# msmbuilder/msmbuilder

Hardware: AMD Instinct MI355X
Metric: frames/sec tICA fit + KCenters assign, 10M x 512 feats (higher is better)
Workload: dtype f32

## Files before the change

### msmbuilder_amd/csrc/distance_kcbatch_dev.h

```cpp
#pragma once
#include "common.h"
#include "distance_dev.h"

namespace msm {

constexpr int KCB_JMAX = 32, KCB_CAP = 2048, KCB_NLEV = 6, KCB_TARGET = 1536;
template <int CTRL>
__device__ __forceinline__ double kcb_dpp_f64(double v)
{
    const int lo = __builtin_amdgcn_update_dpp(0, __double2loint(v), CTRL, 0xf, 0xf, false);
    const int hi = __builtin_amdgcn_update_dpp(0, __double2hiint(v), CTRL, 0xf, 0xf, false);
    return __hiloint2double(hi, lo);
}
__device__ __forceinline__ double kcb_readlane_f64(double v, int lane)
{
    return __hiloint2double(__builtin_amdgcn_readlane(__double2hiint(v), lane), __builtin_amdgcn_readlane(__double2loint(v), lane));
}
__device__ __forceinline__ void kcb_wave_argmax(double v, long long i, double& ov, long long& oi)
{
    const double w = i >= 0 ? v : -1.0;
    double x = w;
    x = fmax(x, kcb_dpp_f64<0xB1>(x));
    x = fmax(x, kcb_dpp_f64<0x4E>(x));
    x = fmax(x, kcb_dpp_f64<0x141>(x));
// ... 163 lines not shown
        }
        if (th > vl) th = vl;
        S->theta = th;
        S->count = 0;
        for (int q = 0; q < KCB_NLEV; ++q) S->lev[q] = 0;
        S->J = J;
        S->k_done = k0 + J;
        S->rounds += 1;
        S->fallbacks += fell;
    }
}

constexpr int KCB_CAPR = 1024, KCB_HDR = 48, KCB_LEV0 = 32;
__host__ __device__ constexpr size_t kcb_rec_doubles(long long m) { return (size_t)KCB_HDR + (size_t)KCB_CAPR * (size_t)(2 + m); }

__global__ void kcb_boot_records_kernel(const double* __restrict__ cands, int world, long long m, double* __restrict__ recs)
{
    const int r = blockIdx.x, tid = threadIdx.x;
    if (r >= world) return;
    const double* c = cands + (size_t)r * (2 + m);
    double* o = recs + (size_t)r * kcb_rec_doubles(m);
    if (tid < KCB_HDR) {
        double v = 0.0;
        if (tid == 8) v = c[0];
        else if (tid == 9) v = c[1];
        else if (tid >= 10 && tid < 10 + 16) v = tid - 10 < m ? c[2 + tid - 10] : 0.0;
        o[tid] = v;
    }
}

template <int NP>
__global__ __launch_bounds__(DT) void kcb_pack_kernel(KscArgs P, KcbState* S, double* __restrict__ rec)
{
    __shared__ double rv[DT];
    __shared__ long long ri[DT];
    const int tid = threadIdx.x, m = (int)P.m;
    if (S->J == 0) return;
    double bv = -1.0;
    long long bi = -1;
    for (int k = tid; k < P.nblk; k += DT) {
        const KcPartial q = P.next[k];
        if (q.i >= 0 && (bi < 0 || kc_better(q.v, q.i, bv, bi))) {
            bv = q.v;
            bi = q.i;
        }
    }
    rv[tid] = bv;
    ri[tid] = bi;
    __syncthreads();
    for (int k = DT / 2; k > 0; k >>= 1) {
        if (tid < k) {
            const long long oi = ri[tid + k];
            if (oi >= 0 && (ri[tid] < 0 || kc_better(rv[tid + k], oi, rv[tid], ri[tid]))) {
                rv[tid] = rv[tid + k];
                ri[tid] = oi;
            }
        }
        __syncthreads();
    }
    const long long w = ri[0];
    const unsigned cnt = S->count;
    if (tid < KCB_HDR) {
        double v = 0.0;
        if (tid == 0) v = (double)cnt;
        else if (tid > KCB_LEV0 && tid < KCB_LEV0 + KCB_NLEV) v = (double)S->lev[tid - KCB_LEV0];
        else if (tid == 8) v = w >= 0 ? rv[0] : -1.0;
        else if (tid == 9) v = w >= 0 ? (double)(P.row_offset + w) : -1.0;
        else if (tid >= 10 && tid < 26) v = (w >= 0 && tid - 10 < m) ? P.X[w * P.m + (tid - 10)] : 0.0;
        rec[tid] = v;
    }
    const unsigned ne = cnt <= (unsigned)KCB_CAPR ? cnt : 0u;
    for (unsigned e = tid; e < ne; e += DT) {
        const long long p = S->list[e];
        double* o = rec + KCB_HDR + (size_t)e * (2 + m);
        o[0] = P.dist[p];
        o[1] = (double)(P.row_offset + p);
        for (int f = 0; f < m; ++f) o[2 + f] = P.X[p * P.m + f];
    }
}

template <int NP>
__global__ __launch_bounds__(DT) void kcenters_batch_pass_kernel(KscArgs P, KcbState* S)
{
    constexpr int R = 2;
    constexpr int NW = ksc_words(NP, 2), RW = NW + 1;
    constexpr int SB = 2 * NP;
    typedef float f32x2 __attribute__((ext_vector_type(2)));
    __shared__ __attribute__((aligned(16))) f32x2 ycf[KCB_JMAX][NP];
    __shared__ double yd[KCB_JMAX][2 * NP];
    __shared__ float epsb[KCB_JMAX];
    __shared__ double rv[DT];
    __shared__ long long ri[DT];
    __shared__ unsigned slev[KCB_NLEV];
    const int tid = threadIdx.x, m = (int)P.m;
    const int J = S->J;
    if (J == 0) return;
    const int kbase = S->k_done - J;
    const float theta = S->theta;
    const long long ntile = (P.n + (long long)R * DT - 1) / ((long long)R * DT);
    unsigned qn[R][RW];
    auto load_tile = [&](long long t) {
#pragma unroll
        for (int k = 0; k < R; ++k) {
            const long long p0 = t * (R * DT) + k * DT + tid;
            const long long pc = p0 < P.n ? p0 : P.n - 1;
            const unsigned* xr = static_cast<const unsigned*>(P.xs) + pc * RW;
            if ((RW & 3) == 0) {
#pragma unroll
                for (int j = 0; j < RW / 4; ++j) {
                    const uint4 v = reinterpret_cast<const uint4*>(xr)[j];
                    qn[k][4 * j] = v.x;
                    qn[k][4 * j + 1] = v.y;
                    qn[k][4 * j + 2] = v.z;
                    qn[k][4 * j + 3] = v.w;
                }
            } else if ((RW & 1) == 0) {
#pragma unroll
                for (int j = 0; j < RW / 2; ++j) {
                    const uint2 v = reinterpret_cast<const uint2*>(xr)[j];
                    qn[k][2 * j] = v.x;
                    qn[k][2 * j + 1] = v.y;
                }
            } else {
#pragma unroll
                for (int j = 0; j < RW; ++j) qn[k][j] = xr[j];
            }
        }
    };
    if ((long long)blockIdx.x < ntile) load_tile(blockIdx.x);
    if (tid < KCB_NLEV) slev[tid] = 0;
    for (int e = tid; e < KCB_JMAX * 2 * NP; e += DT) {
        const int j = e / (2 * NP), f = e - j * (2 * NP);
        const double y = j < J ? S->cen[j][f] : 0.0;
        yd[j][f] = y;
        reinterpret_cast<float*>(&ycf[j][0])[f] = (float)(y - (f < m ? P.c0[f] : 0.0));
    }
    if (tid < KCB_JMAX) {
        double c0n2 = 0.0, yn2 = 0.0, ycn2 = 0.0;
        for (int f = 0; f < 2 * NP; ++f) {
            const double y = tid < J ? S->cen[tid][f] : 0.0, c0f = f < m ? P.c0[f] : 0.0;
            c0n2 = fma(c0f, c0f, c0n2);
            yn2 = fma(y, y, yn2);
            ycn2 = fma(y - c0f, y - c0f, ycn2);
        }
        const double g2 = __longlong_as_double((long long)P.gmax2[0]), r2 = __longlong_as_double((long long)P.gmax2[1]);
        double eps0 = (sqrt(r2) + sqrt(yn2) + 2.0 * sqrt(c0n2)) * 0x1p-48 + 1e-37;
        if (!(g2 < 1e36) || !(r2 < 1e76) || !(ycn2 < 1e36)) eps0 = NAN;
        epsb[tid] = fmaf(0x1p-19f, (float)(sqrt(ycn2) * 1.000001), (float)(eps0 * 1.000001));
    }
    __syncthreads();
    constexpr float E32 = 0x1p-19f;
    constexpr float QSQ = NP == 1 ? 1.4143f : NP == 2 ? 2.f : NP == 3 ? 2.4495f : NP == 4 ? 2.8285f : NP == 5 ? 3.1623f
                        : NP == 6 ? 3.4642f : NP == 7 ? 3.7417f : 4.f;
    constexpr float QA = 0.51f * 1.02f * QSQ + E32 * 127.f * QSQ * 1.001f;
    float bf = -1.f;
    long long bi = -1;
    double bx = 0.0;
    bool bknown = false;
    unsigned nlev[KCB_NLEV];
#pragma unroll
    for (int l = 0; l < KCB_NLEV; ++l) nlev[l] = 0;
    for (long long t = blockIdx.x; t < ntile; t += gridDim.x) {
        float cf[R];
        unsigned cmask[R];
        long long pr[R];
        unsigned q[R][RW];
#pragma unroll
        for (int k = 0; k < R; ++k) {
            pr[k] = t * (R * DT) + k * DT + tid;
#pragma unroll
            for (int j = 0; j < RW; ++j) q[k][j] = qn[k][j];
            cf[k] = __uint_as_float(q[k][NW]);
        }
        if (t + gridDim.x < ntile) load_tile(t + gridDim.x);
#pragma unroll
        for (int k = 0; k < R; ++k) {
            const float sf = __uint_as_float(((q[k][SB >> 2] >> (8 * (SB & 3))) & 0xffffu) << 16);
            f32x2 xt[NP];
#pragma unroll
            for (int g = 0; g < NP; ++g) {
                xt[g].x = (float)((int)(q[k][(2 * g) >> 2] << (24 - 8 * ((2 * g) & 3))) >> 24) * sf;
                xt[g].y = (float)((int)(q[k][(2 * g + 1) >> 2] << (24 - 8 * ((2 * g + 1) & 3))) >> 24) * sf;
            }
            const float base = cf[k] + sf * QA;
            unsigned mk = 0;
            for (int j = 0; j < J; ++j) {
                f32x2 acc = {0.f, 0.f};
#pragma unroll
                for (int g = 0; g < NP; ++g) {
                    const f32x2 d = xt[g] - ycf[j][g];
                    acc = __builtin_elementwise_fma(d, d, acc);
                }
                const float T = (base + epsb[j]) * (1.f + 0x1p-20f);
                if (!(acc.x + acc.y >= T * T)) mk |= 1u << j;
            }
            cmask[k] = pr[k] < P.n ? mk : 0u;
        }
        if (cmask[0] | cmask[1]) {
            double x[R][2 * NP], cur[R];
#pragma unroll
            for (int k = 0; k < R; ++k) {
                const long long pc = pr[k] < P.n ? pr[k] : P.n - 1;
                const double* xp = P.X + pc * P.m;
                if (P.vecw == 16 && (m & 1) == 0) {
#pragma unroll
                    for (int j = 0; j < NP; ++j) {
                        const raw_f32x4 v = *reinterpret_cast<const raw_f32x4*>(xp + 2 * j);
                        x[k][2 * j] = reinterpret_cast<const double*>(&v)[0];
                        x[k][2 * j + 1] = reinterpret_cast<const double*>(&v)[1];
                    }
                } else {
#pragma unroll
                    for (int f = 0; f < 2 * NP; ++f) x[k][f] = xp[f < m ? f : m - 1];
#pragma unroll
                    for (int f = 0; f < 2 * NP; ++f)
                        if (f >= m) x[k][f] = 0.0;
                }
                cur[k] = P.dist[pc];
            }
#pragma unroll
            for (int k = 0; k < R; ++k) {
                unsigned mk = cmask[k];
                int lab = -1;
                double c = cur[k];
                while (mk) {
                    const int j = __builtin_ctz(mk);
                    mk &= mk - 1;
                    double a = 0.0, b = 0.0;
#pragma unroll
                    for (int f = 0; f < 2 * NP; ++f) m_update<double, M_EUCLIDEAN>(a, b, x[k][f], yd[j][f]);
                    const double d = m_final<M_EUCLIDEAN>(a, b, P.m);
                    if (d < c) {
                        c = d;
                        lab = kbase + j;
                    }
                }
                if (lab >= 0) {
                    P.dist[pr[k]] = c;
                    P.labels[pr[k]] = lab;
                    cf[k] = ksc_round_up(c);
                    static_cast<unsigned*>(P.xs)[pr[k] * RW + NW] = __float_as_uint(cf[k]);
                }
            }
        }
#pragma unroll
        for (int k = 0; k < R; ++k) {
            const long long p = pr[k];
            const bool in = p < P.n;
            const bool lst = in && cf[k] > theta;
            const unsigned long long bal = __builtin_amdgcn_ballot_w64(lst);
            if (bal) {
                const int lane = tid & 63, leader = __builtin_ctzll(bal);
                unsigned base = 0;
                if (lane == leader) base = atomicAdd(&S->count, (unsigned)__builtin_popcountll(bal));
                base = __shfl(base, leader);
                if (lst) {
                    const unsigned slot = base + (unsigned)__builtin_popcountll(bal & ((1ull << lane) - 1ull));
                    if (slot < (unsigned)KCB_CAP) S->list[slot] = p;
                }
            }
#pragma unroll
            for (int l = 1; l < KCB_NLEV; ++l) nlev[l] += (in && cf[k] > theta * kcb_level(l)) ? 1u : 0u;
            if (in) {
                if (cf[k] > bf || bi < 0) {
                    bf = cf[k];
                    bi = p;
                    bknown = false;
                } else if (cf[k] == bf) {
                    if (!bknown) {
                        bx = P.dist[bi];
                        bknown = true;
                    }
                    const double v = P.dist[p];
                    if (v > bx) {
                        bx = v;
                        bi = p;
                    }
                }
            }
        }
    }
#pragma unroll
    for (int l = 1; l < KCB_NLEV; ++l)
        if (nlev[l]) atomicAdd(&slev[l], nlev[l]);
    double bvx = -1.0;
    if (bi >= 0) bvx = bknown ? bx : P.dist[bi];
    rv[tid] = bvx;
    ri[tid] = bi;
    __syncthreads();
    if (tid >= 1 && tid < KCB_NLEV && slev[tid]) atomicAdd(&S->lev[tid], slev[tid]);
    for (int k = DT / 2; k > 0; k >>= 1) {
        if (tid < k) {
            const long long oi = ri[tid + k];
            if (oi >= 0 && (ri[tid] < 0 || kc_better(rv[tid + k], oi, rv[tid], ri[tid]))) {
                rv[tid] = rv[tid + k];
                ri[tid] = oi;
            }
        }
        __syncthreads();
    }
    if (tid == 0) {
        KcPartial q;
        q.v = rv[0];
        q.i = ri[0];
        P.next[blockIdx.x] = q;
    }
}

__global__ void kcb_empty_record_kernel(double* __restrict__ rec)
{
    if (threadIdx.x < KCB_HDR) rec[threadIdx.x] = (threadIdx.x == 8 || threadIdx.x == 9) ? -1.0 : 0.0;
}

template <int NP>
__global__ __launch_bounds__(1024) void kcb_select_sharded_kernel(const double* __restrict__ recs, int world, long long mm, KcbState* S, int K,
                                                                   double* __restrict__ cen_out, msm_idx_t* __restrict__ ids_out)
{
    __shared__ double rv[1024];
    __shared__ long long ri[1024];
    __shared__ double cs[16];
    const int tid = threadIdx.x, m = (int)mm;
    const size_t RD = kcb_rec_doubles(mm);
    const int k0 = S->k_done;
    if (k0 >= K) {
        if (tid == 0) S->J = 0;
        return;
    }
// ... 155 lines not shown
```

### msmbuilder_amd/csrc/distance_kcpass_dev.h

```cpp
#pragma once
#include "common.h"
#include "distance_dev.h"

namespace msm {

struct KcPartial {
    double v;
    long long i;
};

struct KcArgs {
    const void* X;
    long long n, m;
    int it;
    long long seed;
    const KcPartial* prev;
    KcPartial* next;
    int nblk;
    double* dist;
    msm_idx_t* labels;
    msm_idx_t* ids;
    int vecw;
    const void* ycenter;
    const void* centers;
    int prune;
    const double* sel_cands;
    int sel_world;
    void* sel_centers;
    msm_idx_t* sel_ids;
    double* cand_out;
    long long row_offset;
    unsigned* counter;
};

constexpr int KC_PRUNE_MAX = 2048;
template <typename T> struct PruneMargin;
template <> struct PruneMargin<double> { static constexpr double F = 2.0 * (1.0 + 1e-9); };
template <> struct PruneMargin<float> { static constexpr double F = 2.0 * (1.0 + 1e-5); };
template <int M> struct IsNormMetric { static constexpr bool V = (M == M_EUCLIDEAN || M == M_CITYBLOCK || M == M_CHEBYSHEV); };

__device__ __forceinline__ bool kc_better(double v, long long i, double bv, long long bi)
{
    return (v > bv) || (v == bv && i < bi);
}

template <typename T, int M, bool REG>
__global__ __launch_bounds__(DT) void kcenters_pass_kernel(KcArgs P)
{
    constexpr int FC = FeatChunk<T>::FC;
    __shared__ T Xs[REG ? 1 : DT * (FC + 1)];
    __shared__ T ys[FC];
    __shared__ double rv[DT];
    __shared__ long long ri[DT];
    const T* X = static_cast<const T*>(P.X);
    const int tid = threadIdx.x;

    long long cidx = 0;
    __shared__ int sel_win;
    if (P.sel_cands) {
        const long long rec = 2 + P.m;
        if (tid == 0) {
            int w = -1;
            for (int r = 0; r < P.sel_world; ++r) {
                const double v = P.sel_cands[r * rec], g = P.sel_cands[r * rec + 1];
                if (g < 0.0) continue;
                if (w < 0 || v > P.sel_cands[w * rec] || (v == P.sel_cands[w * rec] && g < P.sel_cands[w * rec + 1])) w = r;
            }
            sel_win = w;
            if (blockIdx.x == 0) P.sel_ids[P.it] = w >= 0 ? (msm_idx_t)P.sel_cands[w * rec + 1] : -1;
        }
        __syncthreads();
        if (tid < FC) {
            const T v = (tid < P.m && sel_win >= 0) ? (T)P.sel_cands[sel_win * rec + 2 + tid] : (T)0;
            ys[tid] = v;
            if (blockIdx.x == 0 && tid < P.m) static_cast<T*>(P.sel_centers)[(long long)P.it * P.m + tid] = v;
        }
        __syncthreads();
    } else if (P.ycenter) {
    } else if (P.it == 0) {
        cidx = P.seed;
    } else {
        double bv = -1.0;
        long long bi = 0x7fffffffffffffffLL;
        for (int k = tid; k < P.nblk; k += DT) {
            const KcPartial q = P.prev[k];
// ... 95 lines not shown
            double cur = (P.it == 0) ? INFINITY : P.dist[i];
            const bool upd = d < cur;
            if (upd) cur = d;
            if (P.it == 0 || upd) {
                P.dist[i] = cur;
                P.labels[i] = upd ? P.it : 0;
            }
            if (bi < 0 || kc_better(cur, i, bv, bi)) {
                bv = cur;
                bi = i;
            }
        }
    }
    rv[tid] = bv;
    ri[tid] = bi;
    __syncthreads();
    for (int s = DT / 2; s > 0; s >>= 1) {
        if (tid < s) {
            const long long oi = ri[tid + s];
            if (oi >= 0 && (ri[tid] < 0 || kc_better(rv[tid + s], oi, rv[tid], ri[tid]))) {
                rv[tid] = rv[tid + s];
                ri[tid] = oi;
            }
        }
        __syncthreads();
    }
    if (tid == 0) {
        KcPartial q;
        q.v = rv[0];
        q.i = ri[0];
        if (P.cand_out) {
            __hip_atomic_store(&P.next[blockIdx.x].v, q.v, __ATOMIC_RELAXED, __HIP_MEMORY_SCOPE_AGENT);
            __hip_atomic_store(&P.next[blockIdx.x].i, q.i, __ATOMIC_RELAXED, __HIP_MEMORY_SCOPE_AGENT);
            __builtin_amdgcn_fence(__ATOMIC_RELEASE, "agent");
            asm volatile("s_waitcnt vmcnt(0)" ::: "memory");
        } else {
            P.next[blockIdx.x] = q;
        }
    }
    if (P.cand_out) {
        __shared__ int am_last;
        if (tid == 0) {
            const unsigned prev = __hip_atomic_fetch_add(P.counter, 1u, __ATOMIC_RELAXED, __HIP_MEMORY_SCOPE_AGENT);
            am_last = prev == gridDim.x - 1;
            if (am_last) __builtin_amdgcn_fence(__ATOMIC_ACQUIRE, "agent");
        }
        __syncthreads();
        if (am_last) {
            double cv = -1.0;
            long long ci = -1;
            for (int k = tid; k < (int)gridDim.x; k += DT) {
                KcPartial q;
                q.v = __hip_atomic_load(&P.next[k].v, __ATOMIC_RELAXED, __HIP_MEMORY_SCOPE_AGENT);
                q.i = __hip_atomic_load(&P.next[k].i, __ATOMIC_RELAXED, __HIP_MEMORY_SCOPE_AGENT);
                if (q.i >= 0 && (ci < 0 || kc_better(q.v, q.i, cv, ci))) {
                    cv = q.v;
                    ci = q.i;
                }
            }
            rv[tid] = cv;
            ri[tid] = ci;
            __syncthreads();
            for (int s = DT / 2; s > 0; s >>= 1) {
                if (tid < s) {
                    const long long oi = ri[tid + s];
                    if (oi >= 0 && (ri[tid] < 0 || kc_better(rv[tid + s], oi, rv[tid], ri[tid]))) {
                        rv[tid] = rv[tid + s];
                        ri[tid] = oi;
                    }
                }
                __syncthreads();
            }
            const long long w = ri[0];
            if (tid == 0) {
                P.cand_out[0] = w >= 0 ? rv[0] : -1.0;
                P.cand_out[1] = w >= 0 ? (double)(P.row_offset + w) : -1.0;
                __hip_atomic_store(P.counter, 0u, __ATOMIC_RELAXED, __HIP_MEMORY_SCOPE_AGENT);
            }
            for (long long f = tid; f < P.m; f += DT) P.cand_out[2 + f] = w >= 0 ? (double)X[w * P.m + f] : 0.0;
        }
    }
}

struct WideArgs;
template <typename T, int M, int MODE, int NC>
__device__ __forceinline__ void wide_group_end(const WideArgs& A, double (&a)[NC], double (&b)[NC], long long i,
                                               long long j0, long long n, long long m, long long K, double& min_d,
                                               long long& lab);
template <typename T, int M, int MODE>
__device__ __forceinline__ void wide_tile_end(const WideArgs& A, long long i, long long n, double& min_d,
                                              long long& lab, double& inertia, double& bv, long long& bi);
template <typename T, int M, int MODE, int NC>
__device__ __forceinline__ void wide_group_end_split(const WideArgs& A, double (&a)[NC], double (&b)[NC], long long i,
                                                     long long j0, int hh, long long n, long long m, long long K,
                                                     double& min_d, long long& lab, double& min_d2, long long& lab2,
                                                     double* rv, long long* ri);

}
```

### msmbuilder_amd/csrc/distance_screen_dev.h

```cpp
#pragma once
#include "common.h"
#include "distance_dev.h"

namespace msm {

struct KscArgs {
    const double* X;
    void* xs;
    float* curf;
    unsigned long long* gmax2;
    double* c0;
    long long n, m;
    int it, nblk, vecw;
    long long seed;
    const KcPartial* prev;
    KcPartial* next;
    double* dist;
    msm_idx_t* labels;
    msm_idx_t* ids;
    const double* sel_cands;
    int sel_world;
    double* sel_centers;
    msm_idx_t* sel_ids;
    double* cand_out;
    long long row_offset;
    unsigned* counter;
};

__device__ __forceinline__ float ksc_round_up(double c)
{
    float f = (float)c;
    if ((double)f < c) f = __uint_as_float(__float_as_uint(f) + 1u);
    return f;
}

__device__ __forceinline__ unsigned ksc_bf16_rne(float f)
{
    const unsigned u = __float_as_uint(f);
    if ((u & 0x7f800000u) == 0x7f800000u) return u >> 16;
    return (u + 0x7fffu + ((u >> 16) & 1u)) >> 16;
}

constexpr int ksc_words(int np, int fmt) { return fmt == 0 ? 2 * np : fmt == 1 ? np : (2 * np + 2 + 3) / 4; }
__device__ __forceinline__ unsigned ksc_bf16_up(float f)
{
    return (__float_as_uint(f) + 0xffffu) >> 16;
}

template <int NP, int FMT>
__global__ __launch_bounds__(DT) void kcenters_screen_pass_kernel(KscArgs P)
{
    constexpr bool BF16 = FMT == 1;
    constexpr int FC = FeatChunk<double>::FC;
    constexpr int R = 2;
    __shared__ double ys[FC];
    __shared__ double rv[DT];
    __shared__ long long ri[DT];
    const int tid = threadIdx.x;
    const int m = (int)P.m;

    constexpr int NW = ksc_words(NP, FMT);
    constexpr int RW = NW + 1;
    const long long ntile = (P.n + (long long)R * DT - 1) / ((long long)R * DT);
    unsigned qn[R][RW];
    auto load_tile = [&](long long t) {
#pragma unroll
        for (int k = 0; k < R; ++k) {
            const long long p0 = t * (R * DT) + k * DT + tid;
            const long long pc = p0 < P.n ? p0 : P.n - 1;
            const unsigned* xr = static_cast<const unsigned*>(P.xs) + pc * RW;
            if ((RW & 3) == 0) {
#pragma unroll
                for (int j = 0; j < RW / 4; ++j) {
                    const uint4 v = reinterpret_cast<const uint4*>(xr)[j];
                    qn[k][4 * j] = v.x;
                    qn[k][4 * j + 1] = v.y;
                    qn[k][4 * j + 2] = v.z;
                    qn[k][4 * j + 3] = v.w;
                }
            } else if ((RW & 1) == 0) {
#pragma unroll
                for (int j = 0; j < RW / 2; ++j) {
                    const uint2 v = reinterpret_cast<const uint2*>(xr)[j];
                    qn[k][2 * j] = v.x;
                    qn[k][2 * j + 1] = v.y;
                }
            } else {
#pragma unroll
                for (int j = 0; j < RW; ++j) qn[k][j] = xr[j];
            }
        }
    };
    if ((long long)blockIdx.x < ntile) load_tile(blockIdx.x);

    if (P.sel_cands) {
        __shared__ int sel_win;
        const long long rec = 2 + P.m;
        if (tid == 0) {
            int w = -1;
            for (int r = 0; r < P.sel_world; ++r) {
                const double v = P.sel_cands[r * rec], g = P.sel_cands[r * rec + 1];
                if (g < 0.0) continue;
                if (w < 0 || v > P.sel_cands[w * rec] || (v == P.sel_cands[w * rec] && g < P.sel_cands[w * rec + 1])) w = r;
            }
            sel_win = w;
            if (blockIdx.x == 0) P.sel_ids[P.it] = w >= 0 ? (msm_idx_t)P.sel_cands[w * rec + 1] : -1;
        }
        __syncthreads();
        if (tid < FC) {
            const double v = (tid < m && sel_win >= 0) ? P.sel_cands[sel_win * rec + 2 + tid] : 0.0;
            ys[tid] = v;
            if (blockIdx.x == 0 && tid < m) P.sel_centers[(long long)P.it * P.m + tid] = v;
        }
        __syncthreads();
    } else {
    double fv = -1.0;
    long long fi = 0x7fffffffffffffffLL;
    {
        KcPartial q[KC_MAXBLK / DT];
#pragma unroll
        for (int j = 0; j < KC_MAXBLK / DT; ++j) {
            const int k = tid + j * DT;
            q[j] = P.prev[k < P.nblk ? k : P.nblk - 1];
        }
#pragma unroll
        for (int j = 0; j < KC_MAXBLK / DT; ++j) {
            const int k = tid + j * DT;
            if (k < P.nblk && q[j].i >= 0 && kc_better(q[j].v, q[j].i, fv, fi)) {
                fv = q[j].v;
                fi = q[j].i;
// ... 200 lines not shown
        if (tid == 0) {
            const unsigned prev = __hip_atomic_fetch_add(P.counter, 1u, __ATOMIC_RELAXED, __HIP_MEMORY_SCOPE_AGENT);
            am_last = prev == gridDim.x - 1;
            if (am_last) __builtin_amdgcn_fence(__ATOMIC_ACQUIRE, "agent");
        }
        __syncthreads();
        if (am_last) {
            double cv = -1.0;
            long long ci = -1;
            for (int k = tid; k < (int)gridDim.x; k += DT) {
                KcPartial q;
                q.v = __hip_atomic_load(&P.next[k].v, __ATOMIC_RELAXED, __HIP_MEMORY_SCOPE_AGENT);
                q.i = __hip_atomic_load(&P.next[k].i, __ATOMIC_RELAXED, __HIP_MEMORY_SCOPE_AGENT);
                if (q.i >= 0 && (ci < 0 || kc_better(q.v, q.i, cv, ci))) {
                    cv = q.v;
                    ci = q.i;
                }
            }
            rv[tid] = cv;
            ri[tid] = ci;
            __syncthreads();
            for (int s = DT / 2; s > 0; s >>= 1) {
                if (tid < s) {
                    const long long oi = ri[tid + s];
                    if (oi >= 0 && (ri[tid] < 0 || kc_better(rv[tid + s], oi, rv[tid], ri[tid]))) {
                        rv[tid] = rv[tid + s];
                        ri[tid] = oi;
                    }
                }
                __syncthreads();
            }
            const long long w = ri[0];
            if (tid == 0) {
                P.cand_out[0] = w >= 0 ? rv[0] : -1.0;
                P.cand_out[1] = w >= 0 ? (double)(P.row_offset + w) : -1.0;
                __hip_atomic_store(P.counter, 0u, __ATOMIC_RELAXED, __HIP_MEMORY_SCOPE_AGENT);
            }
            for (long long f = tid; f < P.m; f += DT) P.cand_out[2 + f] = w >= 0 ? P.X[w * P.m + f] : 0.0;
        }
    }
}

template <int NP, int FMT>
__global__ __launch_bounds__(DT) void ksc_convert_kernel(KscArgs P)
{
    constexpr bool BF16 = FMT == 1;
    __shared__ double rv[DT];
    __shared__ double rw[DT];
    const int tid = threadIdx.x, m = (int)P.m;
    constexpr int NW = ksc_words(NP, FMT);
    double c0[2 * NP];
#pragma unroll
    for (int f = 0; f < 2 * NP; ++f) c0[f] = f < m ? P.c0[f] : 0.0;
    double gloc = 0.0, rloc = 0.0;
    for (long long p = (long long)blockIdx.x * DT + tid; p < P.n; p += (long long)gridDim.x * DT) {
        const double* x = P.X + p * P.m;
        unsigned* xo = static_cast<unsigned*>(P.xs) + p * (NW + 1);
        double n2 = 0.0, r2 = 0.0;
        float xc[2 * NP];
        double xv[2 * NP], xd[2 * NP];
        if (P.vecw == 16 && (m & 1) == 0) {
#pragma unroll
            for (int j = 0; j < NP; ++j) {
                const raw_f32x4 q = *reinterpret_cast<const raw_f32x4*>(x + 2 * j);
                xv[2 * j] = reinterpret_cast<const double*>(&q)[0];
                xv[2 * j + 1] = reinterpret_cast<const double*>(&q)[1];
            }
        } else {
#pragma unroll
            for (int f = 0; f < 2 * NP; ++f) xv[f] = x[f < m ? f : m - 1];
        }
#pragma unroll
        for (int f = 0; f < 2 * NP; ++f) {
            const double v = xv[f];
            const double c = f < m ? v - c0[f] : 0.0;
            xc[f] = (float)c;
            xd[f] = c;
            if (f < m) {
                n2 = fma(c, c, n2);
                r2 = fma(v, v, r2);
            }
        }
        if (FMT == 2) {
            double smax = 0.0;
            bool bad = false;
#pragma unroll
            for (int f = 0; f < 2 * NP; ++f) {
                const double a = fabs(xd[f]);
                bad = bad || !(a == a);
                smax = a > smax ? a : smax;
            }
            unsigned sbits = 0;
            if (bad || !(smax < 1e37) || (smax > 0.0 && smax < 1e-30)) {
                sbits = 0x7fc0u;
            } else if (smax > 0.0) {
                sbits = ksc_bf16_up((float)(smax * (1.0000002 / 127.0)));
            }
            const double sfd = (double)__uint_as_float(sbits << 16);
            unsigned w[NW];
#pragma unroll
            for (int j = 0; j < NW; ++j) w[j] = 0u;
#pragma unroll
            for (int f = 0; f < 2 * NP; ++f) {
                int qi = 0;
                if (sbits != 0 && sbits != 0x7fc0u) {
                    const double t = rint(xd[f] / sfd);
                    qi = (int)(t > 127.0 ? 127.0 : t < -127.0 ? -127.0 : t);
                }
                w[f >> 2] |= ((unsigned)qi & 0xffu) << (8 * (f & 3));
            }
            w[(2 * NP) >> 2] |= sbits << (8 * ((2 * NP) & 3));
#pragma unroll
            for (int j = 0; j < NW; ++j) xo[j] = w[j];
        } else
#pragma unroll
        for (int j = 0; j < NP; ++j) {
            if (BF16) {
                xo[j] = ksc_bf16_rne(xc[2 * j]) | (ksc_bf16_rne(xc[2 * j + 1]) << 16);
            } else {
                xo[2 * j] = __float_as_uint(xc[2 * j]);
                xo[2 * j + 1] = __float_as_uint(xc[2 * j + 1]);
            }
        }
        if (gloc == gloc && (n2 > gloc || n2 != n2)) gloc = n2;
        if (rloc == rloc && (r2 > rloc || r2 != r2)) rloc = r2;
        xo[NW] = __float_as_uint(ksc_round_up(P.dist[p]));
    }
    const unsigned long long gb = (gloc == gloc) ? (unsigned long long)__double_as_longlong(gloc) : 0x7ff8000000000000ull;
    const unsigned long long rb = (rloc == rloc) ? (unsigned long long)__double_as_longlong(rloc) : 0x7ff8000000000000ull;
    rv[tid] = __longlong_as_double((long long)gb);
    rw[tid] = __longlong_as_double((long long)rb);
    __syncthreads();
    for (int k = DT / 2; k > 0; k >>= 1) {
        if (tid < k) {
            if ((unsigned long long)__double_as_longlong(rv[tid + k]) > (unsigned long long)__double_as_longlong(rv[tid])) rv[tid] = rv[tid + k];
            if ((unsigned long long)__double_as_longlong(rw[tid + k]) > (unsigned long long)__double_as_longlong(rw[tid])) rw[tid] = rw[tid + k];
        }
        __syncthreads();
    }
    if (tid == 0) {
        atomicMax(P.gmax2, (unsigned long long)__double_as_longlong(rv[0]));
        atomicMax(P.gmax2 + 1, (unsigned long long)__double_as_longlong(rw[0]));
    }
}

}
```

### msmbuilder_amd/csrc/kcenters.hip

```cpp
#include "common.h"

#include <algorithm>
#include <cmath>
#include <cstdlib>
#include <vector>

#include "distance_host.h"
#include "distance_kcsel_dev.h"
#include "distance_screen_dev.h"
#include "distance_kcbatch_dev.h"
#include "distance_wscreen_dev.h"
#include "distance_wbatch_dev.h"

namespace msm {

template <typename T>
static bool kc_is_wide(const KcArgs& P) { return P.vecw == 0 && wide_ok<T>(P.X, P.ycenter ? P.ycenter : P.X, P.m, false); }
template <typename T>
static int kc_wide_cut(int nblk, const KcArgs& P) { return kc_is_wide<T>(P) ? std::min(nblk, wide_grid(P.n)) : nblk; }

template <typename T>
void launch_kc(int metric, int grid, const KcArgs& P)
{
    const bool wide = kc_is_wide<T>(P);
// ... 68 lines not shown
    g_kc_stats.rows = n;
    g_kc_stats.plain_row_bytes = (long long)(m * sizeof(T) + 16);
}

struct KcSwitches {
    bool batch;
    bool wscreen;
    int wbatch;
    bool wselect_one;
    bool stats;
};
static KcSwitches kc_switches()
{
    const auto is = [](const char* name, int value) { const char* v = getenv(name); return v && atoi(v) == value; };
    KcSwitches sw;
    sw.batch = !is("MSM_KC_BATCH", 0);
    sw.wscreen = !is("MSM_KC_WSCREEN", 0);
    sw.wbatch = !getenv("MSM_KC_WBATCH") ? -1 : is("MSM_KC_WBATCH", 0) ? 0 : 1;
    sw.wselect_one = is("MSM_KC_WSELECT", 1);
    sw.stats = is("MSM_KC_STATS", 1);
    return sw;
}

static int kc_blocks(long long n) { return (int)std::min<long long>(ceil_div(std::max<long long>(n, 1), DT), KC_MAXBLK); }

struct KcParts {
    KcPartial* base;
    int nblk0;
    KcPartial* next(long long step) const { return base + (size_t)(step & 1) * nblk0; }
    const KcPartial* prev(long long step) const { return next(step + 1); }
    template <typename Args> void aim(Args& A, long long step) const { A.prev = prev(step), A.next = next(step); }
};

template <int NP = 1, typename Fn>
static void ksc_np_visit(int np, Fn&& fn)
{
    if (np == NP) fn(std::integral_constant<int, NP>{});
    else if constexpr (NP < 8) ksc_np_visit<NP + 1>(np, fn);
}

constexpr int KSC_FMT = 2;

struct KscBufs {
    DevBuf xf, curf, misc;
};
static KscBufs& ksc_bufs() { static KscBufs b; return b; }

static int ksc_np(long long m) { return (int)((m + 1) / 2); }
static long long ksc_row_bytes(long long m) { return (long long)(ksc_words(ksc_np(m), KSC_FMT) * 4 + 4); }

static int ksc_open(const KcArgs& P, long long seed, msm_idx_t* ids, bool exchange, KscArgs* S)
{
    KscBufs& B = ksc_bufs();
    int rc;
    if ((rc = B.misc.reserve(64 + 16 * sizeof(double)))) return rc;
    if ((rc = B.xf.reserve((size_t)P.n * (ksc_words(ksc_np(P.m), KSC_FMT) + 1) * sizeof(float)))) return rc;
    MSM_HIP_CHECK(hipMemsetAsync(B.misc.p, 0, 64, stream()));
    memset(S, 0, sizeof(*S));
    S->X = static_cast<const double*>(P.X);
    S->xs = B.xf.p;
    S->gmax2 = B.misc.as<unsigned long long>();
    S->c0 = reinterpret_cast<double*>(static_cast<char*>(B.misc.p) + 64);
    S->n = P.n;
    S->m = P.m;
    S->nblk = P.nblk;
    S->vecw = P.vecw;
    S->seed = seed;
    S->next = P.next;
    S->dist = P.dist;
    S->labels = P.labels;
    S->ids = ids;
    S->row_offset = P.row_offset;
    if (exchange) {
        S->sel_cands = P.sel_cands;
        S->sel_world = P.sel_world;
        S->sel_centers = static_cast<double*>(P.sel_centers);
        S->sel_ids = P.sel_ids;
        S->cand_out = P.cand_out;
        S->counter = P.counter;
    }
    return MSM_OK;
}

static void ksc_queue_copy(const KscArgs& S, const double* centre0)
{
    hipLaunchKernelGGL(ksc_origin_kernel, dim3(1), dim3(64), 0, stream(), S.X, S.ids, (long long)S.m, S.c0, centre0);
    const int gconv = (int)std::min<long long>(ceil_div(S.n, DT), 8LL * num_cus());
    ksc_np_visit(ksc_np(S.m), [&](auto np) {
        hipLaunchKernelGGL((ksc_convert_kernel<decltype(np)::value, KSC_FMT>), dim3(gconv), dim3(DT), 0, stream(), S);
    });
}

static void ksc_queue_pass(const KscArgs& S)
{
    ksc_np_visit(ksc_np(S.m), [&](auto np) {
        hipLaunchKernelGGL((kcenters_screen_pass_kernel<decltype(np)::value, KSC_FMT>), dim3(S.nblk), dim3(DT), 0, stream(), S);
    });
}

static int kcb_group(int K, int done, int rounds_so_far, int done_at_start)
{
    const int left = K - done;
    if (left <= 0) return 0;
    int per = 12;
    if (rounds_so_far > 0) per = std::max(1, (done - done_at_start) / rounds_so_far);
    const int g = (left + per - 1) / per + (rounds_so_far > 0 ? 1 : 0);
    return std::min(std::max(g, 1), 24);
}

template <typename Round, typename Synced = int (*)()>
static int kcb_run_rounds(int K, int done_at_start, KcbState* St, const char* no_progress, Round&& queue_round,
                          Synced synced = [] { return (int)MSM_OK; })
{
    int rc, rounds = 0;
    int head4[4] = {done_at_start, 0, 0, 0};
    while (head4[0] < K) {
        const int group = kcb_group(K, head4[0], rounds, done_at_start);
        for (int r = 0; r < group; ++r, ++rounds)
            if ((rc = queue_round(rounds, r + 1 == group))) return rc;
        MSM_HIP_CHECK(hipGetLastError());
        MSM_HIP_CHECK(hipMemcpyAsync(head4, St, sizeof(head4), hipMemcpyDeviceToHost, stream()));
        MSM_HIP_CHECK(hipStreamSynchronize(stream()));
        if ((rc = synced())) return rc;
        if (rounds > 4 * K) return fail(MSM_ERR_HIP, "%s", no_progress);
    }
    g_kc_stats.screened_passes = head4[2];
    g_kc_stats.batch_fallbacks = head4[3];
    return MSM_OK;
}

template <typename T>
static void kc_run_plain(int mid, KcArgs& P, const KcParts& parts, msm_idx_t first, msm_idx_t last)
{
    for (msm_idx_t it = first; it < last; ++it) {
        P.it = (int)it;
        parts.aim(P, it);
        launch_kc<T>(mid, P.nblk, P);
    }
}

static int kc_run_narrow_screen(int mid, msm_idx_t K, KcArgs& P, const KcParts& parts, const KcSwitches& sw)
{
    const bool kcb_on = sw.batch && P.nblk <= 1024;
    const msm_idx_t probe = kcb_on ? 2 : 4;
    KscArgs S;
    int rc;
    if ((rc = ksc_open(P, P.seed, P.ids, false, &S))) return rc;
    kc_run_plain<double>(mid, P, parts, 0, probe);
    g_kc_stats.plain_passes = probe;
    g_kc_stats.screened_passes = K - probe;
    g_kc_stats.screen_row_bytes = ksc_row_bytes(P.m);
    ksc_queue_copy(S, nullptr);
    if (!kcb_on) {
        for (msm_idx_t it = probe; it < K; ++it) {
            S.it = (int)it;
            parts.aim(S, it);
            ksc_queue_pass(S);
        }
        return MSM_OK;
    }
    DevBuf& SB = pool(PS_W);
    if ((rc = SB.reserve(sizeof(KcbState)))) return rc;
    KcbState* St = SB.as<KcbState>();
    hipLaunchKernelGGL(kcb_init_kernel, dim3(1), dim3(64), 0, stream(), St, (int)probe);
    return kcb_run_rounds((int)K, (int)probe, St, "k-centers: the batched passes made no progress", [&](int round, bool) {
        parts.aim(S, probe + round);
        ksc_np_visit(ksc_np(S.m), [&](auto np) {
            hipLaunchKernelGGL((kcb_select_kernel<decltype(np)::value>), dim3(1), dim3(1024), 0, stream(), S, St, (int)K);
            hipLaunchKernelGGL((kcenters_batch_pass_kernel<decltype(np)::value>), dim3(S.nblk), dim3(DT), 0, stream(), S, St);
        });
        return (int)MSM_OK;
    });
}

struct KwsSizes {
    int kr, gpass;
    int jmax, kr2, gp2;
    int nbsel;
    size_t lds, lds2, ldssel;
};

template <typename T>
static KwsSizes kws_sizes(long long n, long long m, int nb4, int nblk0, const KcSwitches& sw)
{
    KwsSizes Z;
    Z.lds = (size_t)4 * nb4 * sizeof(float) + (size_t)m * sizeof(T);
    Z.kr = nb4 <= 4 ? 8 : nb4 <= 16 ? 4 : 2;
    Z.gpass = (int)std::min<long long>(ceil_div(n, (long long)Z.kr * DT), nblk0);
    Z.jmax = 0;
    {
        const size_t per = (size_t)4 * nb4 * sizeof(float) + ((size_t)m * sizeof(T) + 15) / 16 * 16;
        if (16 * per <= 65536) Z.jmax = 16;
        else if (8 * per <= 65536) Z.jmax = 8;
        const bool pays = (size_t)m * sizeof(T) <= 1024;
        if (sw.wbatch >= 0 ? sw.wbatch == 0 : !pays) Z.jmax = 0;
        Z.lds2 = (size_t)Z.jmax * per;
    }
    Z.kr2 = nb4 <= 16 ? 4 : 2;
    Z.gp2 = (int)std::min<long long>(ceil_div(n, (long long)Z.kr2 * DT), nblk0);
    Z.nbsel = 0;
    Z.ldssel = 0;
    const size_t pitch = (size_t)(m | 1), cpad = (size_t)((m + 3) & ~3LL);
    for (int nb = 8; nb <= 64 && !sw.wselect_one; nb += 8) {
        const size_t rpw = (size_t)ceil_div(KCB_CAP, nb);
        const size_t bytes = (cpad + rpw * pitch) * sizeof(T);
        if (rpw <= (size_t)DT && bytes <= 150000) {
            Z.nbsel = nb;
            Z.ldssel = bytes;
            break;
        }
    }
    return Z;
}

template <typename T>
static int kc_run_wide_screen(int mid, msm_idx_t K, KcArgs& P, const KcParts& parts, const KcSwitches& sw)
{
    constexpr msm_idx_t KWS_PROBE = 4;
    const long long n = P.n, m = P.m;
    const int nblk = P.nblk;
    const int nb4 = (int)((m + 3) / 4);
    const KwsSizes Z = kws_sizes<T>(n, m, nb4, parts.nblk0, sw);
    kc_run_plain<T>(mid, P, parts, 0, KWS_PROBE);
    KscBufs& B = ksc_bufs();
    int rc;
    const size_t qbytes = (size_t)nb4 * n * sizeof(unsigned);
    if ((rc = B.xf.reserve(qbytes + (size_t)n * sizeof(float) + (size_t)n * sizeof(unsigned short) + 64))) return rc;
    if ((rc = B.misc.reserve(64 + (size_t)m * sizeof(double)))) return rc;
    MSM_HIP_CHECK(hipMemsetAsync(B.misc.p, 0, 64, stream()));
    KwsArgs S;
    memset(&S, 0, sizeof(S));
    S.X = P.X;
    S.q = B.xf.as<unsigned>();
    S.curf = reinterpret_cast<float*>(static_cast<char*>(B.xf.p) + qbytes);
    S.sf = reinterpret_cast<unsigned short*>(static_cast<char*>(B.xf.p) + qbytes + (size_t)n * sizeof(float));
// ... 527 lines not shown
```

Measured before the change: 175.4 million.

## Fuse last plain pass with screen copy; rework batch screen to dot-product form

The batch pass kernel now handles four rows per thread instead of two, packed into f32x2 pairs. It computes the screen test as a dot product against pre-scaled centres (-2y), using a precomputed row norm and centre norm plus an added rounding slack term. Separately, the last plain k-centers pass is fused with the quantised copy into a new kernel, so the data is not read a second time by a separate convert kernel. The origin kernel is queued first, and the shared quantisation and reduction helpers move into a common header. This trades register pressure and a looser screen bound for less memory traffic and more arithmetic reuse across centres.

```diff
diff --git a/msmbuilder_amd/csrc/distance_kcbatch_dev.h b/msmbuilder_amd/csrc/distance_kcbatch_dev.h
--- a/msmbuilder_amd/csrc/distance_kcbatch_dev.h
+++ b/msmbuilder_amd/csrc/distance_kcbatch_dev.h
@@ -269,13 +269,13 @@
 template <int NP>
 __global__ __launch_bounds__(DT) void kcenters_batch_pass_kernel(KscArgs P, KcbState* S)
 {
-    constexpr int R = 2;
+    constexpr int R = 4;
     constexpr int NW = ksc_words(NP, 2), RW = NW + 1;
     constexpr int SB = 2 * NP;
+    constexpr int CP = (NP + 1 + 1) & ~1;
     typedef float f32x2 __attribute__((ext_vector_type(2)));
-    __shared__ __attribute__((aligned(16))) f32x2 ycf[KCB_JMAX][NP];
+    __shared__ __attribute__((aligned(16))) f32x2 ycs[KCB_JMAX][CP];
     __shared__ double yd[KCB_JMAX][2 * NP];
-    __shared__ float epsb[KCB_JMAX];
     __shared__ double rv[DT];
     __shared__ long long ri[DT];
     __shared__ unsigned slev[KCB_NLEV];
@@ -320,22 +320,33 @@
         const int j = e / (2 * NP), f = e - j * (2 * NP);
         const double y = j < J ? S->cen[j][f] : 0.0;
         yd[j][f] = y;
-        reinterpret_cast<float*>(&ycf[j][0])[f] = (float)(y - (f < m ? P.c0[f] : 0.0));
+        reinterpret_cast<float*>(&ycs[j][0])[f] = -2.f * (float)(y - (f < m ? P.c0[f] : 0.0));
     }
     if (tid < KCB_JMAX) {
-        double c0n2 = 0.0, yn2 = 0.0, ycn2 = 0.0;
+        double c0n2 = 0.0, yn2 = 0.0, ycn2 = 0.0, yhn2 = 0.0;
         for (int f = 0; f < 2 * NP; ++f) {
             const double y = tid < J ? S->cen[tid][f] : 0.0, c0f = f < m ? P.c0[f] : 0.0;
+            const double yh = (double)(float)(y - c0f);
             c0n2 = fma(c0f, c0f, c0n2);
             yn2 = fma(y, y, yn2);
             ycn2 = fma(y - c0f, y - c0f, ycn2);
+            yhn2 = fma(yh, yh, yhn2);
         }
         const double g2 = __longlong_as_double((long long)P.gmax2[0]), r2 = __longlong_as_double((long long)P.gmax2[1]);
         double eps0 = (sqrt(r2) + sqrt(yn2) + 2.0 * sqrt(c0n2)) * 0x1p-48 + 1e-37;
         if (!(g2 < 1e36) || !(r2 < 1e76) || !(ycn2 < 1e36)) eps0 = NAN;
-        epsb[tid] = fmaf(0x1p-19f, (float)(sqrt(ycn2) * 1.000001), (float)(eps0 * 1.000001));
+        const float ny = yhn2 <= 3e37 ? (float)yhn2 : NAN;
+        const float eps = fmaf(0x1p-19f, (float)(sqrt(ycn2) * 1.000001), (float)(eps0 * 1.000001));
+        ycs[tid][NP] = f32x2{ny, eps};
     }
     __syncthreads();
+    float ynrm = 0.f;
+    for (int j = 0; j < J; ++j) {
+        const float v = ycs[j][NP].x;
+        ynrm = v > ynrm ? v : ynrm;
+    }
+    ynrm = sqrtf(ynrm);
+    constexpr float CE = (float)(2 * NP + 4) * 0x1p-24f * 1.25f;
     constexpr float E32 = 0x1p-19f;
     constexpr float QSQ = NP == 1 ? 1.4143f : NP == 2 ? 2.f : NP == 3 ? 2.4495f : NP == 4 ? 2.8285f : NP == 5 ? 3.1623f
                         : NP == 6 ? 3.4642f : NP == 7 ? 3.7417f : 4.f;
@@ -351,43 +362,62 @@
         float cf[R];
         unsigned cmask[R];
         long long pr[R];
-        unsigned q[R][RW];
-#pragma unroll
-        for (int k = 0; k < R; ++k) {
-            pr[k] = t * (R * DT) + k * DT + tid;
-#pragma unroll
-            for (int j = 0; j < RW; ++j) q[k][j] = qn[k][j];
-            cf[k] = __uint_as_float(q[k][NW]);
-        }
-        if (t + gridDim.x < ntile) load_tile(t + gridDim.x);
-#pragma unroll
-        for (int k = 0; k < R; ++k) {
-            const float sf = __uint_as_float(((q[k][SB >> 2] >> (8 * (SB & 3))) & 0xffffu) << 16);
-            f32x2 xt[NP];
-#pragma unroll
-            for (int g = 0; g < NP; ++g) {
-                xt[g].x = (float)((int)(q[k][(2 * g) >> 2] << (24 - 8 * ((2 * g) & 3))) >> 24) * sf;
-                xt[g].y = (float)((int)(q[k][(2 * g + 1) >> 2] << (24 - 8 * ((2 * g + 1) & 3))) >> 24) * sf;
-            }
-            const float base = cf[k] + sf * QA;
-            unsigned mk = 0;
-            for (int j = 0; j < J; ++j) {
-                f32x2 acc = {0.f, 0.f};
+        f32x2 xt[R / 2][2 * NP], base[R / 2], rowc[R / 2];
+#pragma unroll
+        for (int h = 0; h < R / 2; ++h) {
+            float sf[2];
+#pragma unroll
+            for (int k = 0; k < 2; ++k) {
+                const unsigned* q = qn[2 * h + k];
+                pr[2 * h + k] = t * (R * DT) + (2 * h + k) * DT + tid;
+                cf[2 * h + k] = __uint_as_float(q[NW]);
+                sf[k] = __uint_as_float(((q[SB >> 2] >> (8 * (SB & 3))) & 0xffffu) << 16);
+#pragma unroll
+                for (int f = 0; f < 2 * NP; ++f) xt[h][f][k] = (float)((int)(q[f >> 2] << (24 - 8 * (f & 3))) >> 24) * sf[k];
+            }
+            f32x2 nx = {0.f, 0.f};
+#pragma unroll
+            for (int f = 0; f < 2 * NP; ++f) nx = __builtin_elementwise_fma(xt[h][f], xt[h][f], nx);
+#pragma unroll
+            for (int k = 0; k < 2; ++k) {
+                base[h][k] = cf[2 * h + k] + sf[k] * QA;
+                const float Sp = (sqrtf(nx[k]) + ynrm) * 1.001f;
+                const bool screened = nx[k] <= 3e37f && (sf[k] >= 0x1p-50f || cf[2 * h + k] == 0.f);
+                rowc[h][k] = screened ? nx[k] - CE * Sp * Sp : NAN;
+            }
+        }
+#pragma unroll
+        for (int k = 0; k < R; ++k) cmask[k] = 0u;
+#pragma unroll 1
+        for (int j = 0; j < J; ++j) {
+            f32x2 c[NP + 1];
+#pragma unroll
+            for (int g = 0; g < NP + 1; ++g) c[g] = ycs[j][g];
+            const unsigned bit = 1u << j;
+#pragma unroll
+            for (int h = 0; h < R / 2; ++h) {
+                f32x2 s = c[NP].xx;
 #pragma unroll
                 for (int g = 0; g < NP; ++g) {
-                    const f32x2 d = xt[g] - ycf[j][g];
-                    acc = __builtin_elementwise_fma(d, d, acc);
-                }
-                const float T = (base + epsb[j]) * (1.f + 0x1p-20f);
-                if (!(acc.x + acc.y >= T * T)) mk |= 1u << j;
-            }
-            cmask[k] = pr[k] < P.n ? mk : 0u;
-        }
-        if (cmask[0] | cmask[1]) {
-            double x[R][2 * NP], cur[R];
-#pragma unroll
-            for (int k = 0; k < R; ++k) {
-                const long long pc = pr[k] < P.n ? pr[k] : P.n - 1;
+                    s = __builtin_elementwise_fma(xt[h][2 * g], c[g].xx, s);
+                    s = __builtin_elementwise_fma(xt[h][2 * g + 1], c[g].yy, s);
+                }
+                const f32x2 T = (base[h] + c[NP].yy) * (1.f + 0x1p-20f);
+                const f32x2 lhs = s + rowc[h], T2 = T * T;
+                if (!(lhs.x >= T2.x)) cmask[2 * h] |= bit;
+                if (!(lhs.y >= T2.y)) cmask[2 * h + 1] |= bit;
+            }
+        }
+#pragma unroll
+        for (int k = 0; k < R; ++k)
+            if (!(pr[k] < P.n)) cmask[k] = 0u;
+#pragma unroll
+        for (int h = 0; h < R; h += 2)
+        if (cmask[h] | cmask[h + 1]) {
+            double x[2][2 * NP], cur[2];
+#pragma unroll
+            for (int k = 0; k < 2; ++k) {
+                const long long pc = pr[h + k] < P.n ? pr[h + k] : P.n - 1;
                 const double* xp = P.X + pc * P.m;
                 if (P.vecw == 16 && (m & 1) == 0) {
 #pragma unroll
@@ -406,8 +436,8 @@
                 cur[k] = P.dist[pc];
             }
 #pragma unroll
-            for (int k = 0; k < R; ++k) {
-                unsigned mk = cmask[k];
+            for (int k = 0; k < 2; ++k) {
+                unsigned mk = cmask[h + k];
                 int lab = -1;
                 double c = cur[k];
                 while (mk) {
@@ -423,13 +453,14 @@
                     }
                 }
                 if (lab >= 0) {
-                    P.dist[pr[k]] = c;
-                    P.labels[pr[k]] = lab;
-                    cf[k] = ksc_round_up(c);
-                    static_cast<unsigned*>(P.xs)[pr[k] * RW + NW] = __float_as_uint(cf[k]);
-                }
-            }
-        }
+                    P.dist[pr[h + k]] = c;
+                    P.labels[pr[h + k]] = lab;
+                    cf[h + k] = ksc_round_up(c);
+                    static_cast<unsigned*>(P.xs)[pr[h + k] * RW + NW] = __float_as_uint(cf[h + k]);
+                }
+            }
+        }
+        load_tile(t + gridDim.x < ntile ? t + gridDim.x : t);
 #pragma unroll
         for (int k = 0; k < R; ++k) {
             const long long p = pr[k];
diff --git a/msmbuilder_amd/csrc/distance_kcpass_dev.h b/msmbuilder_amd/csrc/distance_kcpass_dev.h
--- a/msmbuilder_amd/csrc/distance_kcpass_dev.h
+++ b/msmbuilder_amd/csrc/distance_kcpass_dev.h
@@ -1,6 +1,7 @@
 #pragma once
 #include "common.h"
 #include "distance_dev.h"
+#include "distance_kscopy_dev.h"
 
 namespace msm {
 
@@ -262,6 +263,135 @@
     }
 }
 
+template <int NP>
+__global__ __launch_bounds__(DT) void kcenters_pass_copy_kernel(KcArgs P, KscCopyOut O)
+{
+    constexpr int FC = FeatChunk<double>::FC;
+    constexpr int NW = ksc_words(NP, 2);
+    __shared__ double ys[FC];
+    __shared__ double rv[DT];
+    __shared__ long long ri[DT];
+    const double* X = static_cast<const double*>(P.X);
+    const int tid = threadIdx.x, m = (int)P.m;
+    {
+        double bv = -1.0;
+        long long bi = 0x7fffffffffffffffLL;
+        for (int k = tid; k < P.nblk; k += DT) {
+            const KcPartial q = P.prev[k];
+            if (q.i >= 0 && kc_better(q.v, q.i, bv, bi)) {
+                bv = q.v;
+                bi = q.i;
+            }
+        }
+        rv[tid] = bv;
+        ri[tid] = bi;
+        __syncthreads();
+        for (int s = DT / 2; s > 0; s >>= 1) {
+            if (tid < s && kc_better(rv[tid + s], ri[tid + s], rv[tid], ri[tid])) {
+                rv[tid] = rv[tid + s];
+                ri[tid] = ri[tid + s];
+            }
+            __syncthreads();
+        }
+    }
+    const long long cidx = ri[0];
+    __syncthreads();
+    if (blockIdx.x == 0 && tid == 0) P.ids[P.it] = cidx;
+    if (tid < FC) ys[tid] = tid < m ? X[cidx * P.m + tid] : 0.0;
+    __syncthreads();
+    double yr[2 * NP], c0[2 * NP];
+#pragma unroll
+    for (int f = 0; f < 2 * NP; ++f) {
+        yr[f] = ys[f];
+        c0[f] = f < m ? O.c0[f] : 0.0;
+    }
+    double bv = -1.0, gloc = 0.0, rloc = 0.0;
+    long long bi = -1;
+    const long long ntile = (P.n + DT - 1) / DT;
+    for (long long t = blockIdx.x; t < ntile; t += gridDim.x) {
+        const long long i = t * DT + tid;
+        if (i >= P.n) continue;
+        const double* x = X + i * P.m;
+        double xv[2 * NP];
+        if (P.vecw == 16 && (m & 1) == 0) {
+#pragma unroll
+            for (int j = 0; j < NP; ++j) {
+                const raw_f32x4 q = *reinterpret_cast<const raw_f32x4*>(x + 2 * j);
+                xv[2 * j] = reinterpret_cast<const double*>(&q)[0];
+                xv[2 * j + 1] = reinterpret_cast<const double*>(&q)[1];
+            }
+        } else {
+#pragma unroll
+            for (int f = 0; f < 2 * NP; ++f) xv[f] = x[f < m ? f : m - 1];
+#pragma unroll
+            for (int f = 0; f < 2 * NP; ++f)
+                if (f >= m) xv[f] = 0.0;
+        }
+        double cur = P.dist[i];
+        double a = 0.0, b = 0.0;
+#pragma unroll
+        for (int f = 0; f < 2 * NP; ++f) m_update<double, M_EUCLIDEAN>(a, b, xv[f], yr[f]);
+        const double d = m_final<M_EUCLIDEAN>(a, b, P.m);
+        if (d < cur) {
+            cur = d;
+            P.dist[i] = d;
+            P.labels[i] = P.it;
+        }
+        if (bi < 0 || kc_better(cur, i, bv, bi)) {
+            bv = cur;
+            bi = i;
+        }
+        double xd[2 * NP], n2 = 0.0, r2 = 0.0;
+#pragma unroll
+        for (int f = 0; f < 2 * NP; ++f) {
+            const double v = xv[f];
+            const double c = f < m ? v - c0[f] : 0.0;
+            xd[f] = c;
+            if (f < m) {
+                n2 = fma(c, c, n2);
+                r2 = fma(v, v, r2);
+            }
+        }
+        unsigned w[NW];
+        ksc_q8_row<NP>(xd, w);
+        unsigned* xo = static_cast<unsigned*>(O.xs) + i * (NW + 1);
+        const unsigned cw = __float_as_uint(ksc_round_up(cur));
+        unsigned row[NW + 1];
+#pragma unroll
+        for (int j = 0; j < NW; ++j) row[j] = w[j];
+        row[NW] = cw;
+        if (((NW + 1) & 3) == 0) {
+#pragma unroll
+            for (int j = 0; j < (NW + 1) / 4; ++j) reinterpret_cast<uint4*>(xo)[j] = make_uint4(row[4 * j], row[4 * j + 1], row[4 * j + 2], row[4 * j + 3]);
+        } else {
+#pragma unroll
+            for (int j = 0; j < NW + 1; ++j) xo[j] = row[j];
+        }
+        ksc_track_max(gloc, rloc, n2, r2);
+    }
+    rv[tid] = bv;
+    ri[tid] = bi;
+    __syncthreads();
+    for (int s = DT / 2; s > 0; s >>= 1) {
+        if (tid < s) {
+            const long long oi = ri[tid + s];
+            if (oi >= 0 && (ri[tid] < 0 || kc_better(rv[tid + s], oi, rv[tid], ri[tid]))) {
+                rv[tid] = rv[tid + s];
+                ri[tid] = oi;
+            }
+        }
+        __syncthreads();
+    }
+    if (tid == 0) {
+        KcPartial q;
+        q.v = rv[0];
+        q.i = ri[0];
+        P.next[blockIdx.x] = q;
+    }
+    __syncthreads();
+    ksc_reduce_max(gloc, rloc, rv, reinterpret_cast<double*>(ri), O.gmax2);
+}
+
 struct WideArgs;
 template <typename T, int M, int MODE, int NC>
 __device__ __forceinline__ void wide_group_end(const WideArgs& A, double (&a)[NC], double (&b)[NC], long long i,
diff --git a/msmbuilder_amd/csrc/distance_kscopy_dev.h b/msmbuilder_amd/csrc/distance_kscopy_dev.h
--- /dev/null
+++ b/msmbuilder_amd/csrc/distance_kscopy_dev.h
@@ -0,0 +1,85 @@
+#pragma once
+#include "common.h"
+#include "distance_dev.h"
+
+namespace msm {
+
+__device__ __forceinline__ float ksc_round_up(double c)
+{
+    float f = (float)c;
+    if ((double)f < c) f = __uint_as_float(__float_as_uint(f) + 1u);
+    return f;
+}
+
+constexpr int ksc_words(int np, int fmt) { return fmt == 0 ? 2 * np : fmt == 1 ? np : (2 * np + 2 + 3) / 4; }
+__device__ __forceinline__ unsigned ksc_bf16_up(float f)
+{
+    return (__float_as_uint(f) + 0xffffu) >> 16;
+}
+
+struct KscCopyOut {
+    void* xs;
+    unsigned long long* gmax2;
+    const double* c0;
+};
+
+template <int NP>
+__device__ __forceinline__ void ksc_q8_row(const double (&xd)[2 * NP], unsigned (&w)[ksc_words(NP, 2)])
+{
+    constexpr int NW = ksc_words(NP, 2);
+    double smax = 0.0;
+    bool bad = false;
+#pragma unroll
+    for (int f = 0; f < 2 * NP; ++f) {
+        const double a = fabs(xd[f]);
+        bad = bad || !(a == a);
+        smax = a > smax ? a : smax;
+    }
+    unsigned sbits = 0;
+    if (bad || !(smax < 1e37) || (smax > 0.0 && smax < 1e-30)) {
+        sbits = 0x7fc0u;
+    } else if (smax > 0.0) {
+        sbits = ksc_bf16_up((float)(smax * (1.0000002 / 127.0)));
+    }
+    const double sfd = (double)__uint_as_float(sbits << 16);
+#pragma unroll
+    for (int j = 0; j < NW; ++j) w[j] = 0u;
+#pragma unroll
+    for (int f = 0; f < 2 * NP; ++f) {
+        int qi = 0;
+        if (sbits != 0 && sbits != 0x7fc0u) {
+            const double t = rint(xd[f] / sfd);
+            qi = (int)(t > 127.0 ? 127.0 : t < -127.0 ? -127.0 : t);
+        }
+        w[f >> 2] |= ((unsigned)qi & 0xffu) << (8 * (f & 3));
+    }
+    w[(2 * NP) >> 2] |= sbits << (8 * ((2 * NP) & 3));
+}
+
+__device__ __forceinline__ void ksc_track_max(double& gloc, double& rloc, double n2, double r2)
+{
+    if (gloc == gloc && (n2 > gloc || n2 != n2)) gloc = n2;
+    if (rloc == rloc && (r2 > rloc || r2 != r2)) rloc = r2;
+}
+__device__ __forceinline__ void ksc_reduce_max(double gloc, double rloc, double* rv, double* rw, unsigned long long* gmax2)
+{
+    const int tid = threadIdx.x;
+    const unsigned long long gb = (gloc == gloc) ? (unsigned long long)__double_as_longlong(gloc) : 0x7ff8000000000000ull;
+    const unsigned long long rb = (rloc == rloc) ? (unsigned long long)__double_as_longlong(rloc) : 0x7ff8000000000000ull;
+    rv[tid] = __longlong_as_double((long long)gb);
+    rw[tid] = __longlong_as_double((long long)rb);
+    __syncthreads();
+    for (int k = DT / 2; k > 0; k >>= 1) {
+        if (tid < k) {
+            if ((unsigned long long)__double_as_longlong(rv[tid + k]) > (unsigned long long)__double_as_longlong(rv[tid])) rv[tid] = rv[tid + k];
+            if ((unsigned long long)__double_as_longlong(rw[tid + k]) > (unsigned long long)__double_as_longlong(rw[tid])) rw[tid] = rw[tid + k];
+        }
+        __syncthreads();
+    }
+    if (tid == 0) {
+        atomicMax(gmax2, (unsigned long long)__double_as_longlong(rv[0]));
+        atomicMax(gmax2 + 1, (unsigned long long)__double_as_longlong(rw[0]));
+    }
+}
+
+}
diff --git a/msmbuilder_amd/csrc/distance_screen_dev.h b/msmbuilder_amd/csrc/distance_screen_dev.h
--- a/msmbuilder_amd/csrc/distance_screen_dev.h
+++ b/msmbuilder_amd/csrc/distance_screen_dev.h
@@ -1,6 +1,7 @@
 #pragma once
 #include "common.h"
 #include "distance_dev.h"
+#include "distance_kscopy_dev.h"
 
 namespace msm {
 
@@ -27,13 +28,6 @@
     unsigned* counter;
 };
 
-__device__ __forceinline__ float ksc_round_up(double c)
-{
-    float f = (float)c;
-    if ((double)f < c) f = __uint_as_float(__float_as_uint(f) + 1u);
-    return f;
-}
-
 __device__ __forceinline__ unsigned ksc_bf16_rne(float f)
 {
     const unsigned u = __float_as_uint(f);
@@ -41,11 +35,6 @@
     return (u + 0x7fffu + ((u >> 16) & 1u)) >> 16;
 }
 
-constexpr int ksc_words(int np, int fmt) { return fmt == 0 ? 2 * np : fmt == 1 ? np : (2 * np + 2 + 3) / 4; }
-__device__ __forceinline__ unsigned ksc_bf16_up(float f)
-{
-    return (__float_as_uint(f) + 0xffffu) >> 16;
-}
 
 template <int NP, int FMT>
 __global__ __launch_bounds__(DT) void kcenters_screen_pass_kernel(KscArgs P)
@@ -412,34 +401,8 @@
             }
         }
         if (FMT == 2) {
-            double smax = 0.0;
-            bool bad = false;
-#pragma unroll
-            for (int f = 0; f < 2 * NP; ++f) {
-                const double a = fabs(xd[f]);
-                bad = bad || !(a == a);
-                smax = a > smax ? a : smax;
-            }
-            unsigned sbits = 0;
-            if (bad || !(smax < 1e37) || (smax > 0.0 && smax < 1e-30)) {
-                sbits = 0x7fc0u;
-            } else if (smax > 0.0) {
-                sbits = ksc_bf16_up((float)(smax * (1.0000002 / 127.0)));
-            }
-            const double sfd = (double)__uint_as_float(sbits << 16);
             unsigned w[NW];
-#pragma unroll
-            for (int j = 0; j < NW; ++j) w[j] = 0u;
-#pragma unroll
-            for (int f = 0; f < 2 * NP; ++f) {
-                int qi = 0;
-                if (sbits != 0 && sbits != 0x7fc0u) {
-                    const double t = rint(xd[f] / sfd);
-                    qi = (int)(t > 127.0 ? 127.0 : t < -127.0 ? -127.0 : t);
-                }
-                w[f >> 2] |= ((unsigned)qi & 0xffu) << (8 * (f & 3));
-            }
-            w[(2 * NP) >> 2] |= sbits << (8 * ((2 * NP) & 3));
+            ksc_q8_row<NP>(xd, w);
 #pragma unroll
             for (int j = 0; j < NW; ++j) xo[j] = w[j];
         } else
@@ -452,26 +415,10 @@
                 xo[2 * j + 1] = __float_as_uint(xc[2 * j + 1]);
             }
         }
-        if (gloc == gloc && (n2 > gloc || n2 != n2)) gloc = n2;
-        if (rloc == rloc && (r2 > rloc || r2 != r2)) rloc = r2;
+        ksc_track_max(gloc, rloc, n2, r2);
         xo[NW] = __float_as_uint(ksc_round_up(P.dist[p]));
     }
-    const unsigned long long gb = (gloc == gloc) ? (unsigned long long)__double_as_longlong(gloc) : 0x7ff8000000000000ull;
-    const unsigned long long rb = (rloc == rloc) ? (unsigned long long)__double_as_longlong(rloc) : 0x7ff8000000000000ull;
-    rv[tid] = __longlong_as_double((long long)gb);
-    rw[tid] = __longlong_as_double((long long)rb);
-    __syncthreads();
-    for (int k = DT / 2; k > 0; k >>= 1) {
-        if (tid < k) {
-            if ((unsigned long long)__double_as_longlong(rv[tid + k]) > (unsigned long long)__double_as_longlong(rv[tid])) rv[tid] = rv[tid + k];
-            if ((unsigned long long)__double_as_longlong(rw[tid + k]) > (unsigned long long)__double_as_longlong(rw[tid])) rw[tid] = rw[tid + k];
-        }
-        __syncthreads();
-    }
-    if (tid == 0) {
-        atomicMax(P.gmax2, (unsigned long long)__double_as_longlong(rv[0]));
-        atomicMax(P.gmax2 + 1, (unsigned long long)__double_as_longlong(rw[0]));
-    }
+    ksc_reduce_max(gloc, rloc, rv, rw, P.gmax2);
 }
 
 }
diff --git a/msmbuilder_amd/csrc/kcenters.hip b/msmbuilder_amd/csrc/kcenters.hip
--- a/msmbuilder_amd/csrc/kcenters.hip
+++ b/msmbuilder_amd/csrc/kcenters.hip
@@ -174,9 +174,14 @@
     return MSM_OK;
 }
 
+static void ksc_queue_origin(const KscArgs& S, const double* centre0)
+{
+    hipLaunchKernelGGL(ksc_origin_kernel, dim3(1), dim3(64), 0, stream(), S.X, S.ids, (long long)S.m, S.c0, centre0);
+}
+
 static void ksc_queue_copy(const KscArgs& S, const double* centre0)
 {
-    hipLaunchKernelGGL(ksc_origin_kernel, dim3(1), dim3(64), 0, stream(), S.X, S.ids, (long long)S.m, S.c0, centre0);
+    ksc_queue_origin(S, centre0);
     const int gconv = (int)std::min<long long>(ceil_div(S.n, DT), 8LL * num_cus());
     ksc_np_visit(ksc_np(S.m), [&](auto np) {
         hipLaunchKernelGGL((ksc_convert_kernel<decltype(np)::value, KSC_FMT>), dim3(gconv), dim3(DT), 0, stream(), S);
@@ -238,11 +243,17 @@
     KscArgs S;
     int rc;
     if ((rc = ksc_open(P, P.seed, P.ids, false, &S))) return rc;
-    kc_run_plain<double>(mid, P, parts, 0, probe);
+    ksc_queue_origin(S, S.X + P.seed * P.m);
+    kc_run_plain<double>(mid, P, parts, 0, probe - 1);
+    P.it = (int)(probe - 1);
+    parts.aim(P, probe - 1);
+    const KscCopyOut O = {S.xs, S.gmax2, S.c0};
+    ksc_np_visit(ksc_np(P.m), [&](auto np) {
+        hipLaunchKernelGGL((kcenters_pass_copy_kernel<decltype(np)::value>), dim3(P.nblk), dim3(DT), 0, stream(), P, O);
+    });
     g_kc_stats.plain_passes = probe;
     g_kc_stats.screened_passes = K - probe;
     g_kc_stats.screen_row_bytes = ksc_row_bytes(P.m);
-    ksc_queue_copy(S, nullptr);
     if (!kcb_on) {
         for (msm_idx_t it = probe; it < K; ++it) {
             S.it = (int)it;
```

Result: no change. 177.0 million (median of 6 runs) (+0.9%).
